# cvg/limap

Hardware: AMD Instinct MI355X
Metric: 3D line candidates scored/sec (100 views x 500 segs per GPU, matched topk=10) (higher is better)
Workload: dtype f64

## Files before the change

limap_amd/csrc/lt_api.cpp:

```cpp

#include "lt_host.h"

using namespace lt;
using namespace lt_impl;

namespace lt_trace {
typedef int (*push_fn)(const char *);
typedef int (*pop_fn)(void);
static push_fn g_push = nullptr;
static pop_fn g_pop = nullptr;
static void init_once() {
  static bool done = false;
  if (done) return;
  done = true;
  const char *sw = getenv("LT_ROCTX");
  if (sw && sw[0] == '0') return;
  const char *libs[] = {"librocprofiler-sdk-roctx.so.1", "librocprofiler-sdk-roctx.so", "libroctx64.so.4", "libroctx64.so"};
  for (const char *l : libs) {
    void *h = dlopen(l, RTLD_LAZY | RTLD_GLOBAL);
    if (!h) continue;
    g_push = (push_fn)dlsym(h, "roctxRangePushA");
    g_pop = (pop_fn)dlsym(h, "roctxRangePop");
    if (g_push && g_pop) return;
    g_push = nullptr;
// ... 508 lines not shown
                    &ctx->d_seg_off, &ctx->d_node_img, &ctx->d_nb_off, &ctx->d_blk_img, &ctx->d_blk_nb,
                    &ctx->d_blk_slot, &ctx->d_blk_order, &ctx->d_m_off, &ctx->d_m_pairs, &ctx->d_c_stream, &ctx->d_ovf, &ctx->d_rowdesc, &ctx->d_pairs,
                    &ctx->d_keys, &ctx->d_rows, &ctx->d_row_blk, &ctx->d_skeys, &ctx->d_srows, &ctx->d_sort_tmp,
                    &ctx->d_conn_off, &ctx->d_st_c, &ctx->d_st_l, &ctx->d_flags, &ctx->d_pos, &ctx->d_scan_tmp,
                    &ctx->d_item_off, &ctx->d_masks, &ctx->d_mask_cnt, &ctx->d_mask_pos, &ctx->d_cand, &ctx->d_hcand, &ctx->d_hlite,
                    &ctx->d_rm_line, &ctx->d_rm_act, &ctx->d_rm_edges, &ctx->d_rm_cnt,
                    &ctx->d_lite, &ctx->d_tri_off, &ctx->d_score, &ctx->d_best_idx, &ctx->d_edge_flag,
                    &ctx->d_nvalid, &ctx->d_edge_off, &ctx->d_edges, &ctx->d_best_c, &ctx->d_best_score,
                    &ctx->d_best_src, &ctx->d_ntris, &ctx->d_err, &ctx->d_blk_line_base, &ctx->d_cnt_bl,
                    &ctx->d_st_key, &ctx->d_wave_count, &ctx->d_wave_pos, &ctx->d_ntris_u, &ctx->d_cand_node,
                    &ctx->d_pair_counter, &ctx->d_result3, &ctx->d_tile_order, &ctx->d_scan_status, &ctx->d_perm, &ctx->d_rng, &ctx->d_chunks, &ctx->d_cand_meta, &ctx->d_st_row, &ctx->d_surv_count, &ctx->d_seg_gates, &ctx->d_blkrec, &ctx->d_seg_vp, &ctx->d_seg_has_vp, &ctx->d_base_bl, &ctx->d_blk_chunk_off, &ctx->d_needed, &ctx->d_seg_pts, &ctx->d_seg_pt_off, &ctx->d_sfm_xyz,
                    &ctx->d_place_perm, &ctx->d_ex_rec, &ctx->d_ex_ent, &ctx->d_node_rec, &ctx->d_ex_z, &ctx->d_tile_list, &ctx->d_tail_keys, &ctx->d_tail_skeys, &ctx->d_tail_sims, &ctx->d_tail_mark,
                    &ctx->d_tail_pos, &ctx->d_tail_recs, &ctx->d_tail_nodes, &ctx->d_tail_tmp, &ctx->d_tail_keep,
                    &ctx->d_tail_kpos, &ctx->d_sp_slots, &ctx->d_sp_cnt, &ctx->d_sp_ovf, &ctx->d_sp_pairs, &ctx->d_sp_desc,
                    &ctx->d_run_len, &ctx->d_slot_row0, &ctx->d_blk_nruns, &ctx->d_ln_flag, &ctx->d_blk_surv, &ctx->d_blk_rnd0,
                    &ctx->d_round_count};
  lt_host::host_block_release(ctx->h_pinned_blk);
  if (ctx->tail_pend.active) lt_host::host_block_release(ctx->tail_pend.hb);
  if (ctx->ev_tail) (void)hipEventDestroy(ctx->ev_tail);
  lt_host::host_block_release(ctx->best_c_blk);
  lt_host::host_block_release(ctx->init_blk);
  for (DevBuf *b : bufs) b->release();
  for (auto &e : ctx->ev_b)
    if (e) (void)hipEventDestroy(e);
  for (auto &e : ctx->ev_end)
    if (e) (void)hipEventDestroy(e);
  if (ctx->pool_stream) (void)hipStreamSynchronize(ctx->pool_stream);
  if (!(ctx->pool_stream && lt_host::stream_set_release(ctx->device, ctx->pool_stream, ctx->ev))) {
    for (auto &ev : ctx->ev)
      if (ev) (void)hipEventDestroy(ev);
    if (ctx->pool_stream) (void)hipStreamDestroy(ctx->pool_stream);
// ... 302 lines not shown
```

limap_amd/csrc/lt_api_run.cpp:

```cpp
#include "lt_host.h"

using namespace lt;
using namespace lt_impl;

extern "C" {

int lt_upload(lt_ctx *ctx) {
  LT_RANGE("lt_upload (match rows + job tables -> HBM)");
  LT_FINISH(ctx);
  if (!ctx->inited) return fail(ctx, LT_ERR_STATE, "upload before Init");
  if (ctx->uploaded) return LT_OK;
  HIPCHK(ctx, hipSetDevice(ctx->device));
  double t0 = now_ms();
  build_job_tables(ctx);
  ctx->blk_vorder_ok = false;
  int rc;
  {
    std::vector<char> need((size_t)std::max(ctx->n_img, 1), 0);
    for (size_t j = 0; j < ctx->job_imgs.size(); ++j) {
      need[(size_t)ctx->job_imgs[j]] = 1;
      for (int nb : ctx->job_nbs[j]) need[(size_t)nb] = 1;
    }
    std::vector<int> list;
    ctx->max_needed_segs = 0;
// ... 85 lines not shown
    }
    if (!ctx->rows_ln)
      launch_expand_rows(ctx->stream, ctx->n_blk, ctx->d_rowdesc.p, ctx->d_c_stream.as<unsigned>(), ctx->d_ovf.as<unsigned>(),
                         ctx->d_m_pairs.as<unsigned>());
    if ((rc = upload_vec(ctx, ctx->d_m_off, m_off))) return rc;
    {
      std::vector<int> vo((size_t)std::max(ctx->n_blk, 1), 0);
      for (int b = 0; b < ctx->n_blk; ++b) vo[(size_t)b] = b;
      std::stable_sort(vo.begin(), vo.begin() + ctx->n_blk, [&](int x, int y) {
        return ctx->h_blk_nb[(size_t)x] != ctx->h_blk_nb[(size_t)y] ? ctx->h_blk_nb[(size_t)x] < ctx->h_blk_nb[(size_t)y]
                                                                    : ctx->h_blk_img[(size_t)x] < ctx->h_blk_img[(size_t)y];
      });
      if ((rc = upload_vec(ctx, ctx->d_blk_vorder, vo))) return rc;
      ctx->blk_vorder_ok = true;
    }
    ENSURE(ctx, ctx->d_blkrec, blk_rec_bytes() * (size_t)std::max(ctx->n_blk, 1));
    launch_build_blk(ctx->stream, ctx->n_blk, ctx->d_m_off.as<long long>(), ctx->d_blk_img.as<int>(),
                     ctx->d_blk_nb.as<int>(), ctx->d_blk_slot.as<int>(), ctx->d_seg_off.as<long long>(),
                     ctx->d_blk_line_base.as<long long>(), ctx->d_blkrec.p);
  } else if (ctx->job_mode == 2) {
    ctx->h_item_off.assign(ctx->G + 1, 0);
    std::vector<int> blk_chunk_off((size_t)std::max(ctx->n_blk, 1), 0);
    ctx->max_chunks = 1;
    long long items = 0, conns = 0;
    for (int i = 0; i < ctx->n_img; ++i) {
      long long per_node = 0, conn_node = 0;
      for (long long b = ctx->h_nb_off[i]; b < ctx->h_nb_off[i + 1]; ++b) {
        int i2 = ctx->h_blk_nb[b];
        long long M2 = ctx->seg_off[i2 + 1] - ctx->seg_off[i2];
        blk_chunk_off[(size_t)b] = (int)per_node;
        ctx->max_chunks = std::max(ctx->max_chunks, (int)((M2 + 63) / 64));
        per_node += (M2 + 63) / 64;
        conn_node += M2;
      }
// ... 205 lines not shown
    const bool fast = ctx->rows_sorted;
    {
      const bool vp_now = ctx->cfg.use_vp && !ctx->cfg.disable_vp_triangulation;
      const bool pts_now = ctx->pts_ready && (!ctx->cfg.disable_many_points_triangulation || !ctx->cfg.disable_one_point_triangulation);
      if (ctx->rows_ln && (vp_now || pts_now)) {
        launch_expand_rows(st, ctx->n_blk, ctx->d_rowdesc.p, ctx->d_c_stream.as<unsigned>(), ctx->d_ovf.as<unsigned>(),
                           ctx->d_m_pairs.as<unsigned>());
        ctx->rows_ln = false;
      }
    }
    const bool ln = ctx->rows_ln && fast;
    const int ln_slots = ln ? ctx->ln_slots : 0;
    if (ln) ENSURE(ctx, ctx->d_round_count, 4 * (size_t)std::max<long long>(ctx->n_round_slots, 1));
    const long long n_waves = (long long)ctx->n_blk * gen_groups(ctx->max_rows);
    const long long n_slots_all = (long long)ctx->n_blk * (ln ? ln_slots : gen_slots(ctx->max_rows));
    const long long n_entries = ctx->h_blk_line_base[ctx->n_blk];
    const bool vp_on = ctx->cfg.use_vp && !ctx->cfg.disable_vp_triangulation;
    if (vp_on && !ctx->vp_ready) return fail(ctx, LT_ERR_STATE, "use_vp is set but InitVPResults was not called");
    const bool pts_any = ctx->pts_ready && (!ctx->cfg.disable_many_points_triangulation || !ctx->cfg.disable_one_point_triangulation);
    const bool many_on = pts_any && !ctx->cfg.disable_many_points_triangulation;
    const bool one_on = pts_any && !ctx->cfg.disable_one_point_triangulation;
    const bool pts_on = pts_any;
    const bool extras = vp_on || pts_on;
    long long staged_total = -1;
    if (!extras) {
      ENSURE(ctx, ctx->d_st_c, sizeof(CRec) * Pn); ENSURE(ctx, ctx->d_st_l, sizeof(double) * Pn);
      ENSURE(ctx, ctx->d_st_key, 4 * (Pn + 64));
    }
    ENSURE(ctx, ctx->d_wave_count, 4 * (size_t)(n_waves + 1));
    if (extras) ENSURE(ctx, ctx->d_wave_pos, 8 * (size_t)(n_waves + 1));
    const long long *group_base = extras ? ctx->d_wave_pos.as<long long>() : nullptr;
// ... 56 lines not shown
          return fail(ctx, LT_ERR_ARGUMENT, "too many candidates in one batch (>= 2^32-1): triangulate the images in smaller batches");
        const size_t Sn = (size_t)std::max<long long>(staged_total, 1);
        ENSURE(ctx, ctx->d_st_c, sizeof(CRec) * Sn); ENSURE(ctx, ctx->d_st_l, sizeof(double) * Sn);
        ENSURE(ctx, ctx->d_st_key, 4 * Sn);
        gen(2);
      }
    }
    bool gen_event_pending = false;
    if (fine_gen && ctx->n_blk > 0 && ctx->max_rows > 0) ev_gen_end = 10;
    else gen_event_pending = true;
    long long *hC = hp;
    long long hC_fallback = 0;
    if (!hC) hC = &hC_fallback;
    if (fast) {
      ENSURE(ctx, ctx->d_node_rec, 16 * (size_t)std::max<long long>(G, 1));
      launch_node_prefix(st, G, ctx->d_node_img.as<int>(), ctx->d_seg_off.as<long long>(),
                         ctx->d_nb_off.as<long long>(), ctx->d_blk_line_base.as<long long>(),
                         ctx->d_cnt_bl.as<unsigned>(), ctx->d_base_bl.as<unsigned>(), ctx->d_ntris_u.as<unsigned>(),
                         ctx->d_tri_off.as<long long>(), ctx->d_scan_status.as<unsigned long long>(),
                         ctx->d_err.as<int>(), ctx->d_node_rec.p);
      node_rec_valid = true;
      ctx->cnt_bl_clean = true;
      const long long bound = P;
      constexpr long long kCountFreeBytes = 48ll << 30;
      const bool perm_bound = !test_switch("LT_TEST_PLACE_COPY");
      const long long per_cand = (perm_bound ? 4 : (long long)(sizeof(CRec) + 8)) + 8 + 4 + 4 + (long long)cand_meta_bytes() +
                                 (long long)score_split_entry_bytes() * 256 / 64;
      if (extras) {
        C_known = staged_total;
      } else if (ctx->h_pinned && bound * per_cand <= kCountFreeBytes && !test_switch("LT_TEST_SYNC_COUNT")) {
        C_known = -1;
        C_bound = bound;
      } else {
// ... 27 lines not shown
        HIPCHK(ctx, hipMemcpyAsync(hC, ctx->d_tri_off.as<long long>() + G, 8, hipMemcpyDeviceToHost, st));
        HIPCHK(ctx, hipStreamSynchronize(st));
        C_known = *hC;
      }
    }
    if (C_known >= 0) C_bound = C_known;
    const size_t Cn = (size_t)std::max<long long>(C_bound, 1);
    if (perm_mode) {
      ENSURE(ctx, ctx->d_place_perm, 4 * Cn);
    } else {
      ENSURE(ctx, ctx->d_cand, sizeof(CRec) * Cn); ENSURE(ctx, ctx->d_lite, sizeof(double) * Cn);
    }
    ENSURE(ctx, ctx->d_score, 8 * Cn); ENSURE(ctx, ctx->d_edge_flag, 4 * Cn); ENSURE(ctx, ctx->d_cand_node, 4 * Cn);
    ctx->cand_cap = (long long)Cn;
    if (fast) {
      launch_place(st, ctx->n_blk, ctx->max_rows, ctx->d_m_off.as<long long>(), ctx->d_blk_img.as<int>(),
                   ctx->d_seg_off.as<long long>(), ctx->d_blk_line_base.as<long long>(),
                   ctx->d_base_bl.as<unsigned>(), ctx->d_wave_count.as<unsigned>(), ctx->d_tri_off.as<long long>(),
                   ctx->d_st_c.as<CRec>(), ctx->d_st_l.as<double>(), ctx->d_st_key.as<unsigned>(),
                   ctx->d_cand.as<CRec>(), ctx->d_lite.as<double>(), ctx->d_cand_node.as<unsigned>(), group_base,
                   perm_mode ? ctx->d_place_perm.as<unsigned>() : nullptr, ctx->d_blk_surv.as<unsigned>(),
                   ctx->d_blk_rnd0.as<unsigned>(), ln ? ctx->d_round_count.as<unsigned>() : nullptr);
    } else {
      ENSURE(ctx, ctx->d_keys, 4 * Cn); ENSURE(ctx, ctx->d_rows, 4 * Cn);
      ENSURE(ctx, ctx->d_skeys, 4 * Cn); ENSURE(ctx, ctx->d_srows, 4 * Cn);
      launch_pack_keys(st, ctx->n_blk, ctx->max_rows, ctx->d_m_off.as<long long>(),
                       ctx->d_wave_count.as<unsigned>(), ctx->d_wave_pos.as<long long>(),
                       ctx->d_st_key.as<unsigned>(), ctx->d_keys.as<unsigned>(), ctx->d_rows.as<unsigned>(), group_base);
      if (C_known > 0) {
        int end_bit = bits_for(G + 1);
        size_t tmp = sort_temp_bytes(C_known, end_bit);
        ENSURE(ctx, ctx->d_sort_tmp, std::max<size_t>(tmp, 16));
// ... 441 lines not shown
```

limap_amd/csrc/lt_ctx.h:

```cpp
#pragma once

#include "../../include/limap_amd.h"
#include "lt_device.h"

#include <algorithm>
#include <cstdlib>
#include <cstring>
#include <mutex>
#include <string>
#include <hip/hip_runtime.h>
#include <unordered_map>
#include <vector>

namespace lt_host {
using namespace lt;

void *dev_block_acquire(size_t bytes, size_t *cap);
void dev_block_release(void *p, size_t cap);

struct DevBuf {
  void *p = nullptr;
  size_t cap = 0;
  DevBuf() = default;
  DevBuf(const DevBuf &) = delete;
// ... 207 lines not shown
  long long max_needed_segs = 0;
  DevBuf d_blk_chunk_off;
  int max_chunks = 1;
  DevBuf d_perm, d_rng;
  DevBuf d_result3;
  DevBuf d_scan_status;
  DevBuf d_tile_order;
  DevBuf d_tile_list;
  DevBuf d_blk_vorder;
  bool blk_vorder_ok = false;
  DevBuf d_pc_cnt, d_pc_list;
  DevBuf d_sp_slots, d_sp_cnt, d_sp_ovf, d_sp_pairs, d_sp_desc;
  bool score_two_kernels = false;
  bool score_fused = false;
  DevBuf d_base_bl;
  DevBuf d_place_perm;
  bool perm_mode = false;
  DevBuf d_ex_rec;
  DevBuf d_node_rec;
  DevBuf d_ex_ent;
  DevBuf d_ex_z;
  long long ex_region_cap = 0;
  double ex_frac = 0.0;
  bool ex_two_pass = false;
  bool ex_staged_set[2] = {false, false};
  bool in_run_async = false;
  bool pend_fine_gen = false, pend_fine_score = false;
  int ex_retry_depth = 0;
  bool host_view_valid = false;
  bool compact_valid = false;
// ... 140 lines not shown
```

limap_amd/csrc/lt_host.h:

```cpp
#pragma once

#include "lt_ctx.h"
#include "lt_tail.h"
#include "lt_rows.h"
#include "lt_pool.h"

#include <algorithm>
#include <atomic>
#include <parallel/algorithm>
#include <chrono>
#include <cmath>
#include <cstdio>
#include <cstring>
#include <dlfcn.h>
#include <map>
#include <mutex>
#include <queue>
#include <set>
#include <string>
#include <unordered_map>
#include <vector>

namespace lt {
void launch_fn_query(hipStream_t st, const double *in30, int by_endpoints, double *out32);
int gen_slots(long long max_rows);
int gen_groups(long long max_rows);
int gen_slots_ln(int max_own_segs);
int gen_max_run();
void launch_rows_ln(hipStream_t st, int n_blk, int n_slots, const void *desc, const unsigned *stream,
                    const long long *blk_line_base, unsigned *rstart, int *blk_nruns, unsigned *run_len,
                    unsigned *slot_row0, unsigned short *tr, int *ln_flag);
size_t seg_gate_bytes();
void launch_build_blk(hipStream_t st, int n_blk, const long long *m_off, const int *blk_img, const int *blk_nb,
                      const int *blk_slot, const long long *seg_off, const long long *blk_line_base, void *blkrec);
size_t blk_rec_bytes();
void launch_gen_split(hipStream_t st, int n_blk, long long max_rows, const GenCfg &cfg, const long long *m_off,
                      const int *m_pairs, const int *blk_img, const int *blk_nb, const int *blk_slot,
                      const long long *seg_off, const Cam *cams, const Seg *segs, const PairRec *pairs,
                      const long long *blk_line_base, CRec *st_r, double *st_unc, unsigned *st_key,
                      unsigned *wave_count, unsigned *cnt_bl, int lds_segs, int lds_segs1, void *st_row,
                      unsigned *surv_count, long long n_segs, void *gates, void *blkrec, hipEvent_t *ev3,
                      const double *seg_vp, const unsigned char *seg_has_vp, const long long *seg_pt_off,
                      const void *seg_pts, const double *sfm_xyz, int *err_flag, int many_on, int one_on,
                      const long long *group_base, int phase, int ln_slots, const unsigned short *tr,
                      const unsigned *run_len, const unsigned *slot_row0, unsigned *blk_surv, const unsigned *blk_rnd0,
                      unsigned *round_count, const int *blk_vorder, unsigned *tri_unit_ctr);
size_t seg_point_bytes();
void launch_node_prefix(hipStream_t st, long long G, const int *node_img, const long long *seg_off,
                        const long long *nb_off, const long long *blk_line_base, unsigned *cnt_bl,
                        unsigned *base_bl, unsigned *n_tris, long long *tri_off, unsigned long long *status,
                        int *err_flag, void *node_rec);
void launch_expand_rows(hipStream_t st, int n_blk, const void *desc, const unsigned *stream, const unsigned *ovf, unsigned *rows);
void launch_place(hipStream_t st, int n_blk, long long max_rows, const long long *m_off, const int *blk_img,
                  const long long *seg_off, const long long *blk_line_base, const unsigned *base_bl,
                  const unsigned *wave_count, const long long *tri_off, const CRec *st_r, const double *st_unc,
                  const unsigned *st_key, CRec *cand, double *cand_unc, unsigned *cand_node, const long long *group_base,
                  unsigned *perm, const unsigned *blk_surv, const unsigned *blk_rnd0, const unsigned *round_count);
void launch_pack_keys(hipStream_t st, int n_blk, long long max_rows, const long long *m_off,
                      const unsigned *wave_count, const long long *wave_pos, const unsigned *st_key,
                      unsigned *keys_c, unsigned *src_c, const long long *group_base);
void launch_permute(hipStream_t st, long long C, const unsigned *skeys, const unsigned *ssrc, const CRec *st_r,
                    const double *st_unc, CRec *cand, double *cand_unc, unsigned *cand_node);
void launch_host_view(hipStream_t st, long long C, const unsigned *perm, const CRec *rec, const double *unc, Cand *out_c,
                      CandLite *out_l);
void launch_cand_node(hipStream_t st, long long G, const long long *tri_off, unsigned *cand_node);
size_t score3_lds_bytes(int max_nb, bool f32);
size_t cand_meta_bytes();
void launch_score3(hipStream_t st, long long C, long long G, const long long *tri_off, const unsigned *cand_node,
                   void *meta, const CRec *cand, const int *node_img, const long long *nb_off,
// ... 57 lines not shown
```

limap_amd/csrc/lt_kernels_v2.hip:

```cpp

#include "lt_devfn.h"

#include <algorithm>

namespace lt {

#ifndef LT_GEN_CHUNKS
#define LT_GEN_CHUNKS 5
#endif
#ifndef LT_GATE_WAVES
#define LT_GATE_WAVES 8
#endif
#ifndef LT_GATE_WAVES_PER_EU
#define LT_GATE_WAVES_PER_EU 4
#endif
#define LT_GATE_OCC __attribute__((amdgpu_waves_per_eu(LT_GATE_WAVES_PER_EU, LT_GATE_WAVES_PER_EU)))
constexpr int kGenChunks = LT_GEN_CHUNKS;
constexpr int kRowsPerWave = 64 * kGenChunks;
constexpr int kGateWaves = LT_GATE_WAVES;
#ifndef LT_TRI_SLOTS
#define LT_TRI_SLOTS 4
#endif
constexpr int kTriSlots = LT_TRI_SLOTS;
#ifndef LT_TRI_WAVES
// ... 47 lines not shown
  const unsigned *slot_row0;
};
static __device__ __forceinline__ long long slot_first_row(const unsigned *__restrict__ slot_row0, int n_slots, int b, int s,
                                                           long long rb) {
  return slot_row0 ? (long long)slot_row0[(size_t)b * n_slots + s] : rb + (long long)s * kRowsPerWave;
}


struct BlkRec {
  long long rb, re;
  long long g1, g2;
  long long lbase;
  int M2;
  int i1, i2, nbslot;
  int M1;
  int pad_;
};
static_assert(sizeof(BlkRec) == 64, "BlkRec layout");

__global__ void k_build_blk(int n_blk, const long long *__restrict__ m_off, const int *__restrict__ blk_img,
                            const int *__restrict__ blk_nb, const int *__restrict__ blk_slot,
                            const long long *__restrict__ seg_off, const long long *__restrict__ blk_line_base,
                            BlkRec *__restrict__ out) {
  int b = blockIdx.x * blockDim.x + threadIdx.x;
  if (b >= n_blk) return;
  BlkRec r;
  r.rb = m_off[b]; r.re = m_off[b + 1];
  r.i1 = blk_img[b]; r.i2 = blk_nb[b]; r.nbslot = blk_slot[b];
  r.g1 = seg_off[r.i1]; r.g2 = seg_off[r.i2];
  r.M2 = (int)(seg_off[r.i2 + 1] - r.g2);
  r.lbase = blk_line_base[b];
  r.M1 = (int)(seg_off[r.i1 + 1] - r.g1);
  r.pad_ = 0;
  out[b] = r;
}

constexpr int kExpandWaves = 4;
__global__ void __launch_bounds__(64 * kExpandWaves)
k_expand_rows(int n_blk, const RowDesc *__restrict__ desc, const unsigned *__restrict__ stream,
              const unsigned *__restrict__ ovf, unsigned *__restrict__ rows) {
  const int b = blockIdx.x;
  if (b >= n_blk) return;
  const RowDesc d = desc[b];
  const int lane = lane_id();
  const int wave = threadIdx.x >> 6;
  unsigned *out = rows + d.row_off;
  if (d.ooff >= 0) {
    for (int r = threadIdx.x; r < d.n; r += 64 * kExpandWaves) out[r] = ovf[d.ooff + r];
// ... 481 lines not shown
  const int n_groups = a.n_slots / kTS;
  const int g = blockIdx.x * kTriWaves + wave;
  if (g >= n_groups) return;
  const BlkRec *rec = blk_r + b;
  const long long rb = rec->rb, re = rec->re;
  const long long r0 = slot_first_row(slot_row0, a.n_slots, b, g * kTS, rb);
  const unsigned lin = (unsigned)b * (unsigned)n_groups + (unsigned)g;
  LT_TRACE_MARK(1, lin, 0);
  if (r0 >= re) {
    if (lane == 0) a.wave_count[lin] = 0;
    return;
  }
  const int i1 = rec->i1, i2 = rec->i2, nbslot = rec->nbslot;
  const long long g1 = rec->g1, g2 = rec->g2;
  const PairRec *pr = pairs_r + b;
  const long long lbase = a.cnt_bl ? rec->lbase : 0;
  const long long out0 = (kExtra && a.group_base) ? a.group_base[lin] : r0;
  const bool wr = !(kExtra && a.count_only);
  unsigned cs[kTS + 1];
  cs[0] = 0;
#pragma unroll
  for (int k = 0; k < kTS; ++k)
    cs[k + 1] = cs[k] + a.surv_count[(size_t)b * a.n_slots + (size_t)g * kTS + k];
  const unsigned n_s = cs[kTS];
  unsigned wcount = 0;
#ifdef LT_TRACE
  if (n_s > 0) LT_TRACE_MARK(1, lin, 1);
#endif
  for (unsigned e0 = 0; e0 < n_s; e0 += 64) {
    const unsigned e = e0 + lane;
    bool ok = false;
// ... 187 lines not shown
    if (!first) v += v_step;
    if (v >= v_end) break;
  }
  first = false;
  const int b = vorder ? vorder[v] : v;
  const int x = x_dyn >= 0 ? x_dyn : (wave + b) % kTriWaves;
  const unsigned n_s = blk_surv[b];
  const int n_rounds = (int)((n_s + 63u) >> 6);
  if (x >= n_rounds) continue;
  const BlkRec *rec = blk_r + b;
  const long long rb = rec->rb;
  const unsigned rnd0 = blk_rnd0[b];
  const int i1 = rec->i1, i2 = rec->i2, nbslot = rec->nbslot;
  const long long g1 = rec->g1, g2 = rec->g2;
  const PairRec *pr = pairs_r + b;
  const long long lbase = rec->lbase;
  for (int r = x; r < n_rounds; r += kTriWaves) {
    LT_TRACE_MARK(1, rnd0 + (unsigned)r, 0);
    const unsigned e = 64u * (unsigned)r + (unsigned)lane;
    bool ok = false;
    GenOut o;
    int line = 0;
    if (e < n_s) {
      const uint2 u = a.st_row[rb + e];
      line = (int)(u.x & 0x7FFFFFFFu);
      const int ng = (int)u.y;
#ifdef LT_TRACE
      if (line >= 0) LT_TRACE_MARK(1, rnd0 + (unsigned)r, 1);
#endif
      const Seg &s1 = a.segs[g1 + line];
      const Seg &s2 = a.segs[g2 + ng];
// ... 22 lines not shown
    wave_lds_sync();
    const long long p0 = rb + 64ll * r;
    double2 *dc = reinterpret_cast<double2 *>(a.st_r + p0);
    for (unsigned u = lane; u < total * 8u; u += 64) dc[u] = Lc[u];
    if ((unsigned)lane < total) {
      a.st_unc[p0 + lane] = Lu[lane];
      a.st_key[p0 + lane] = Lk[lane];
    }
    if (lane == 0) round_count[rnd0 + (unsigned)r] = total;
    wave_lds_sync();
    LT_TRACE_MARK(1, rnd0 + (unsigned)r, 2);
  }
  }
}

#ifndef LT_PLACE_WG_PER_CU
#define LT_PLACE_WG_PER_CU 8
#endif
__global__ void __launch_bounds__(256)
k_place_rounds(const long long *__restrict__ m_off, const int *__restrict__ blk_img, const long long *__restrict__ seg_off,
               const long long *__restrict__ blk_line_base, const unsigned *__restrict__ base_bl,
               const long long *__restrict__ tri_off, const CRec *__restrict__ st_r, const double *__restrict__ st_unc,
               const unsigned *__restrict__ st_key, CRec *__restrict__ cand, double *__restrict__ cand_unc,
               unsigned *__restrict__ cand_node, unsigned *__restrict__ perm, const unsigned *__restrict__ blk_surv,
               const unsigned *__restrict__ blk_rnd0, const unsigned *__restrict__ round_count, int n_blk) {
  const int wave = threadIdx.x >> 6;
  const int lane = lane_id();
  for (int b = (int)blockIdx.x; b < n_blk; b += (int)gridDim.x) {
  const int x = (wave + b) & 3;
  const int n_rounds = (int)((blk_surv[b] + 63u) >> 6);
  if (x >= n_rounds) continue;
  const long long rb = m_off[b];
  const unsigned rnd0 = blk_rnd0[b];
  const long long g1 = seg_off[blk_img[b]];
  const long long lbase = blk_line_base[b];
  unsigned count_n = round_count[rnd0 + (unsigned)x];
  unsigned key_n = st_key[rb + 64ll * x + lane];
  for (int r = x; r < n_rounds; r += 4) {
    const unsigned count = count_n;
    const unsigned key_raw = key_n;
    if (r + 4 < n_rounds) {
      count_n = round_count[rnd0 + (unsigned)(r + 4)];
      key_n = st_key[rb + 64ll * (r + 4) + lane];
    }
    if (count == 0) continue;
    const long long s0 = rb + 64ll * r;
    const bool act = (unsigned)lane < count;
    const unsigned key = act ? key_raw : 0xFFFFFFFFu;
    const unsigned prev = (unsigned)__shfl_up((int)key, 1);
    const bool head = act && (lane == 0 || key != prev);
    const unsigned long long heads = __ballot(head);
    const int my_head = 63 - __builtin_clzll(heads & ((2ull << lane) - 1ull) | 1ull);
    const unsigned key0 = (unsigned)__builtin_amdgcn_readfirstlane((int)key);
    unsigned carry = 0;
    for (int pr_ = r - 1; pr_ >= 0; --pr_) {
      const unsigned pc = round_count[rnd0 + (unsigned)pr_];
      if (pc == 0) continue;
      const long long j = (long long)pc - 64 + lane;
      const bool valid = j >= 0;
      const unsigned k = valid ? st_key[rb + 64ll * pr_ + j] : 0u;
      const unsigned long long m = __ballot(valid && k == key0);
      const unsigned lead = m == ~0ull ? 64u : (unsigned)__builtin_clzll(~m);
      carry += lead;
      if (lead < pc) break;
    }
    unsigned pos32 = 0;
    if (act) {
      const unsigned rank = (unsigned)(lane - my_head) + (my_head == 0 ? carry : 0u);
      const long long pos = tri_off[key] + base_bl[lbase + (long long)(key - g1)] + rank;
      pos32 = (unsigned)pos;
      cand_node[pos] = key;
      if (perm) perm[pos] = (unsigned)(s0 + lane);
    }
    if (perm) continue;
    const double2 *src_c = reinterpret_cast<const double2 *>(st_r + s0);
    double2 *dst_c = reinterpret_cast<double2 *>(cand);
#pragma unroll
    for (int it = 0; it < 8; ++it) {
      const unsigned u = (unsigned)it * 64u + (unsigned)lane;
      const unsigned ci = u >> 3, piece = u & 7u;
      const unsigned p = (unsigned)__shfl((int)pos32, (int)ci);
      if (u < count * 8u) dst_c[(size_t)p * 8u + piece] = src_c[u];
    }
    if (act) cand_unc[pos32] = st_unc[s0 + lane];
  }
  }
}

__global__ void __launch_bounds__(256)
k_node_prefix(long long G, const int *__restrict__ node_img, const long long *__restrict__ seg_off,
              const long long *__restrict__ nb_off, const long long *__restrict__ blk_line_base,
              unsigned *__restrict__ cnt_bl, unsigned *__restrict__ base_bl, unsigned *__restrict__ n_tris,
              long long *__restrict__ tri_off, unsigned long long *__restrict__ status, int *__restrict__ err_flag,
              uint4 *__restrict__ node_rec) {
  __shared__ unsigned s_tile;
  __shared__ long long s_wave[4];
  __shared__ long long s_prefix;
  if (threadIdx.x == 0) s_tile = (unsigned)atomicAdd(&status[0], 1ull);
  __syncthreads();
  const long long tile = s_tile;
  const long long g = tile * 256 + threadIdx.x;
  const int lane = lane_id(), wave = threadIdx.x >> 6;
  unsigned run = 0;
  unsigned nbv = 0;
  if (g < G) {
    int img = node_img[g];
    int line = (int)(g - seg_off[img]);
    const long long b0 = nb_off[img], b1 = nb_off[img + 1];
    nbv = ((unsigned)b0 << 8) | (unsigned)(b1 - b0);
    for (long long bb = b0; bb < b1; bb += 16) {
      long long e[16];
      unsigned c[16];
#pragma unroll
      for (int k = 0; k < 16; ++k) {
        e[k] = (bb + k < b1) ? blk_line_base[bb + k] + line : -1;
      }
#pragma unroll
      for (int k = 0; k < 16; ++k) c[k] = e[k] >= 0 ? cnt_bl[e[k]] : 0u;
#pragma unroll
      for (int k = 0; k < 16; ++k) {
        if (e[k] >= 0) {
          cnt_bl[e[k]] = 0;
          base_bl[e[k]] = run;
        }
        run += c[k];
      }
    }
  }
  long long incl = (long long)run;
#pragma unroll
  for (int d = 1; d < 64; d <<= 1) {
    const long long o = __shfl_up(incl, d);
    if (lane >= d) incl += o;
  }
  if (lane == 63) s_wave[wave] = incl;
  __syncthreads();
  long long wbase = 0;
  for (int w = 0; w < wave; ++w) wbase += s_wave[w];
// ... 31 lines not shown
      atomicExch(&status[1 + tile], (2ull << 62) | (unsigned long long)(prefix + total));
      s_prefix = prefix;
    }
  }
  __syncthreads();
  const long long off = s_prefix + wbase + incl - (long long)run;
  if (g <= G) {
    tri_off[g] = off;
    n_tris[g] = run;
  }
  if (node_rec && g < G) node_rec[g] = uint4{(unsigned)(off & 0xFFFFFFFFll), (unsigned)(off >> 32), run, nbv};
}

template <int kTS>
__global__ void __launch_bounds__(256)
k_place(const long long *__restrict__ m_off, const int *__restrict__ blk_img,
        const long long *__restrict__ seg_off, const long long *__restrict__ blk_line_base,
        const unsigned *__restrict__ base_bl, const unsigned *__restrict__ wave_count,
        const long long *__restrict__ tri_off, const CRec *__restrict__ st_r,
        const double *__restrict__ st_unc, const unsigned *__restrict__ st_key, CRec *__restrict__ cand,
        double *__restrict__ cand_unc, unsigned *__restrict__ cand_node, int n_groups,
        const long long *__restrict__ group_base, unsigned *__restrict__ perm,
        const unsigned *__restrict__ slot_row0) {
  const int wave = threadIdx.x >> 6;
  const int lane = lane_id();
  const int b = blockIdx.y;
  const int g = blockIdx.x * 4 + wave;
  if (g >= n_groups) return;
  const int n_slots = n_groups * kTS;
  const long long rb = m_off[b], re = m_off[b + 1];
  const long long r0 = slot_first_row(slot_row0, n_slots, b, g * kTS, rb);
  if (r0 >= re) return;
  const unsigned lin = (unsigned)b * (unsigned)n_groups + (unsigned)g;
  const unsigned count = wave_count[lin];
  if (count == 0) return;
  const long long g1 = seg_off[blk_img[b]];
  const long long lbase = blk_line_base[b];
  const long long s0 = group_base ? group_base[lin] : r0;
  static_assert(sizeof(CRec) == 8 * 16, "record size in 16-byte units");
  for (unsigned e0 = 0; e0 < count; e0 += 64) {
    const unsigned e = e0 + lane;
    const bool act = e < count;
    unsigned pos32 = 0;
    const unsigned key = act ? st_key[s0 + e] : 0xFFFFFFFFu;
    const unsigned prev = (unsigned)__shfl_up((int)key, 1);
    const bool head = act && (lane == 0 || key != prev);
    const unsigned long long heads = __ballot(head);
    const int my_head = 63 - __builtin_clzll(heads & ((2ull << lane) - 1ull) | 1ull);
    const unsigned key0 = (unsigned)__builtin_amdgcn_readfirstlane((int)key);
    unsigned carry = 0;
    {
      long long cur_r0 = r0;
// ... 12 lines not shown
          const long long n_valid = idx_end < 64 ? idx_end : 64;
          if ((long long)lead < n_valid) { more = false; break; }
          idx_end -= n_valid;
        }
        if (!more) break;
        if (cur_g == 0) break;
        cur_g -= 1;
        cur_r0 = slot_first_row(slot_row0, n_slots, b, cur_g * kTS, rb);
        cur_lin -= 1;
        idx_end = (long long)wave_count[cur_lin];
      }
    }
    if (act) {
      const unsigned rank = (unsigned)(lane - my_head) + (my_head == 0 ? carry : 0u);
      const long long toff = tri_off[key];
      const long long pos = toff + base_bl[lbase + (long long)(key - g1)] + rank;
      pos32 = (unsigned)pos;
      cand_node[pos] = key;
      if (perm) perm[pos] = (unsigned)(s0 + e);
    }
    if (perm) continue;
    const unsigned nb = min(64u, count - e0);
    const double2 *src_c = reinterpret_cast<const double2 *>(st_r + s0 + e0);
    double2 *dst_c = reinterpret_cast<double2 *>(cand);
#pragma unroll
    for (int it = 0; it < 8; ++it) {
      const unsigned u = (unsigned)it * 64u + (unsigned)lane;
      const unsigned ci = u >> 3, piece = u & 7u;
      const unsigned p = (unsigned)__shfl((int)pos32, (int)ci);
      if (u < nb * 8u) dst_c[(size_t)p * 8u + piece] = src_c[u];
    }
// ... 74 lines not shown
int score_read_trace(unsigned long long *host, size_t n);
extern "C" int lt_debug_read_trace(unsigned long long *host, size_t n) {
  const int rc = (int)hipMemcpyFromSymbol(host, HIP_SYMBOL(g_trace), n * 8, 0, hipMemcpyDeviceToHost);
  return rc ? rc : score_read_trace(host, n);
}
#endif
size_t seg_gate_bytes() { return sizeof(SegGate); }
size_t seg_point_bytes() { return sizeof(SegPoint); }
size_t blk_rec_bytes() { return sizeof(BlkRec); }
void launch_expand_rows(hipStream_t st, int n_blk, const void *desc, const unsigned *stream, const unsigned *ovf, unsigned *rows) {
  if (n_blk > 0)
    hipLaunchKernelGGL(k_expand_rows, dim3((unsigned)n_blk), dim3(64 * kExpandWaves), 0, st, n_blk, reinterpret_cast<const RowDesc *>(desc), stream,
                       ovf, rows);
}
void launch_build_blk(hipStream_t st, int n_blk, const long long *m_off, const int *blk_img, const int *blk_nb,
                      const int *blk_slot, const long long *seg_off, const long long *blk_line_base, void *blkrec) {
  if (n_blk > 0)
    hipLaunchKernelGGL(k_build_blk, dim3(nblk2(n_blk, 128)), dim3(128), 0, st, n_blk, m_off, blk_img, blk_nb, blk_slot,
                       seg_off, blk_line_base, reinterpret_cast<BlkRec *>(blkrec));
}
void launch_gen_split(hipStream_t st, int n_blk, long long max_rows, const GenCfg &cfg, const long long *m_off,
                      const int *m_pairs, const int *blk_img, const int *blk_nb, const int *blk_slot,
                      const long long *seg_off, const Cam *cams, const Seg *segs, const PairRec *pairs,
                      const long long *blk_line_base, CRec *st_r, double *st_unc, unsigned *st_key,
                      unsigned *wave_count, unsigned *cnt_bl, int lds_segs, int lds_segs1, void *st_row,
                      unsigned *surv_count, long long n_segs, void *gates, void *blkrec, hipEvent_t *ev3,
                      const double *seg_vp, const unsigned char *seg_has_vp, const long long *seg_pt_off,
                      const void *seg_pts, const double *sfm_xyz, int *err_flag, int many_on, int one_on,
                      const long long *group_base, int phase, int ln_slots, const unsigned short *tr,
                      const unsigned *run_len, const unsigned *slot_row0, unsigned *blk_surv, const unsigned *blk_rnd0,
                      unsigned *round_count, const int *blk_vorder, unsigned *tri_unit_ctr) {
  if (n_blk <= 0 || max_rows <= 0) return;
  static int n_cu = 0;
  if (n_cu == 0) {
// ... 44 lines not shown
  const size_t tri_lds = kTriWaves * (64 * 9 + 16) * sizeof(double2);
  if (ln) {
    const dim3 tg((unsigned)std::min<long long>(n_blk, (long long)n_cu * (16 / kTriWaves)));
    hipLaunchKernelGGL(k_tri_rounds, tg, dim3(64 * kTriWaves), tri_lds, st, a, cfg, a.cams, a.pairs, a.blk, blk_surv, blk_rnd0,
                       round_count, blk_vorder, tri_unit_ctr);
  } else {
    const dim3 tg(nblk2(a.n_slots / kTriSlots, kTriWaves), n_blk);
    if (extra)
      hipLaunchKernelGGL((k_tri_rows<true, kTriSlots>), tg, dim3(64 * kTriWaves), 0, st, a, cfg, a.cams, a.pairs, a.blk, a.slot_row0);
    else
      hipLaunchKernelGGL((k_tri_rows<false, kTriSlots>), tg, dim3(64 * kTriWaves), tri_lds, st, a, cfg, a.cams, a.pairs, a.blk,
                         a.slot_row0);
  }
  if (ev3 && phase != 1) (void)hipEventRecord(ev3[2], st);
}
void launch_node_prefix(hipStream_t st, long long G, const int *node_img, const long long *seg_off,
                        const long long *nb_off, const long long *blk_line_base, unsigned *cnt_bl,
                        unsigned *base_bl, unsigned *n_tris, long long *tri_off, unsigned long long *status,
                        int *err_flag, void *node_rec) {
  hipLaunchKernelGGL(k_node_prefix, dim3(nblk2(G + 1, 256)), dim3(256), 0, st, G, node_img, seg_off, nb_off,
                     blk_line_base, cnt_bl, base_bl, n_tris, tri_off, status, err_flag, reinterpret_cast<uint4 *>(node_rec));
}
void launch_place(hipStream_t st, int n_blk, long long max_rows, const long long *m_off, const int *blk_img,
                  const long long *seg_off, const long long *blk_line_base, const unsigned *base_bl,
                  const unsigned *wave_count, const long long *tri_off, const CRec *st_r, const double *st_unc,
                  const unsigned *st_key, CRec *cand, double *cand_unc, unsigned *cand_node, const long long *group_base,
                  unsigned *perm, const unsigned *blk_surv, const unsigned *blk_rnd0, const unsigned *round_count) {
  if (n_blk <= 0 || max_rows <= 0) return;
  if (round_count) {
    static int n_cu = 0;
    if (n_cu == 0) {
      int dev = 0;
      if (hipGetDevice(&dev) != hipSuccess ||
          hipDeviceGetAttribute(&n_cu, hipDeviceAttributeMultiprocessorCount, dev) != hipSuccess || n_cu <= 0)
        n_cu = 256;
    }
    hipLaunchKernelGGL(k_place_rounds, dim3((unsigned)std::min<long long>(n_blk, (long long)n_cu * LT_PLACE_WG_PER_CU)), dim3(256), 0, st, m_off,
                       blk_img, seg_off, blk_line_base, base_bl, tri_off, st_r, st_unc, st_key, cand, cand_unc, cand_node, perm,
                       blk_surv, blk_rnd0, round_count, n_blk);
    return;
  }
  const int n_groups = gen_groups(max_rows);
  hipLaunchKernelGGL(k_place<kTriSlots>, dim3(nblk2(n_groups, 4), n_blk), dim3(256), 0, st, m_off, blk_img, seg_off,
                     blk_line_base, base_bl, wave_count, tri_off, st_r, st_unc, st_key, cand, cand_unc, cand_node, n_groups,
                     group_base, perm, (const unsigned *)nullptr);
}
void launch_pack_keys(hipStream_t st, int n_blk, long long max_rows, const long long *m_off,
                      const unsigned *wave_count, const long long *wave_pos, const unsigned *st_key,
                      unsigned *keys_c, unsigned *src_c, const long long *group_base) {
  if (n_blk <= 0 || max_rows <= 0) return;
  const int n_groups = gen_groups(max_rows);
  hipLaunchKernelGGL(k_pack_keys, dim3(nblk2(n_groups, 4), n_blk), dim3(256), 0, st, m_off, wave_count, wave_pos,
                     st_key, keys_c, src_c, n_groups, group_base);
}
void launch_permute(hipStream_t st, long long C, const unsigned *skeys, const unsigned *ssrc, const CRec *st_r,
                    const double *st_unc, CRec *cand, double *cand_unc, unsigned *cand_node) {
  if (C > 0)
    hipLaunchKernelGGL(k_permute, dim3(nblk2(C, 256)), dim3(256), 0, st, C, skeys, ssrc, st_r, st_unc, cand, cand_unc,
                       cand_node);
// ... 7 lines not shown
```

Baseline: 2.500 billion.

## Re-lay per-(neighbour,segment) counters as slot-major strided arrays and restructure placement

Changes the counter/base arrays from per-block line-base layout to a neighbour-slot-major layout with a padded global-segment stride, so node_prefix reads coalesced contiguous columns per slot. A per-node neighbour descriptor is precomputed on the host and uploaded, which drops the indirect node_img/seg_off/nb_off lookups. k_place_rounds moves from a persistent grid-stride loop with 4 waves to one workgroup per block with 16 waves. Each round now prefetches the previous round's keys for the carry computation. The trade-off is a counter buffer sized max_nb*stride, which may be larger than before, plus a new 2^32 limit check.

```diff
diff --git a/limap_amd/csrc/lt_api.cpp b/limap_amd/csrc/lt_api.cpp
--- a/limap_amd/csrc/lt_api.cpp
+++ b/limap_amd/csrc/lt_api.cpp
@@ -546,7 +546,7 @@
                     &ctx->d_tail_pos, &ctx->d_tail_recs, &ctx->d_tail_nodes, &ctx->d_tail_tmp, &ctx->d_tail_keep,
                     &ctx->d_tail_kpos, &ctx->d_sp_slots, &ctx->d_sp_cnt, &ctx->d_sp_ovf, &ctx->d_sp_pairs, &ctx->d_sp_desc,
                     &ctx->d_run_len, &ctx->d_slot_row0, &ctx->d_blk_nruns, &ctx->d_ln_flag, &ctx->d_blk_surv, &ctx->d_blk_rnd0,
-                    &ctx->d_round_count};
+                    &ctx->d_round_count, &ctx->d_node_nbv};
   lt_host::host_block_release(ctx->h_pinned_blk);
   if (ctx->tail_pend.active) lt_host::host_block_release(ctx->tail_pend.hb);
   if (ctx->ev_tail) (void)hipEventDestroy(ctx->ev_tail);
diff --git a/limap_amd/csrc/lt_api_run.cpp b/limap_amd/csrc/lt_api_run.cpp
--- a/limap_amd/csrc/lt_api_run.cpp
+++ b/limap_amd/csrc/lt_api_run.cpp
@@ -123,10 +123,21 @@
       if ((rc = upload_vec(ctx, ctx->d_blk_vorder, vo))) return rc;
       ctx->blk_vorder_ok = true;
     }
+    {
+      ctx->cnt_stride = (std::max<long long>(ctx->G, 1) + 255) & ~255ll;
+      if ((long long)ctx->max_nb * ctx->cnt_stride >= (1ll << 32))
+        return fail(ctx, LT_ERR_ARGUMENT, "too many (neighbour, segment) counters in one batch (>= 2^32): triangulate the images in smaller batches");
+      std::vector<unsigned> nbv((size_t)std::max<long long>(ctx->G, 1), 0u);
+      for (long long g = 0; g < ctx->G; ++g) {
+        const int i = ctx->h_node_img[(size_t)g];
+        nbv[(size_t)g] = ((unsigned)ctx->h_nb_off[i] << 8) | (unsigned)(ctx->h_nb_off[i + 1] - ctx->h_nb_off[i]);
+      }
+      if ((rc = upload_vec(ctx, ctx->d_node_nbv, nbv))) return rc;
+    }
     ENSURE(ctx, ctx->d_blkrec, blk_rec_bytes() * (size_t)std::max(ctx->n_blk, 1));
     launch_build_blk(ctx->stream, ctx->n_blk, ctx->d_m_off.as<long long>(), ctx->d_blk_img.as<int>(),
                      ctx->d_blk_nb.as<int>(), ctx->d_blk_slot.as<int>(), ctx->d_seg_off.as<long long>(),
-                     ctx->d_blk_line_base.as<long long>(), ctx->d_blkrec.p);
+                     ctx->d_blk_line_base.as<long long>(), ctx->cnt_stride, ctx->d_blkrec.p);
   } else if (ctx->job_mode == 2) {
     ctx->h_item_off.assign(ctx->G + 1, 0);
     std::vector<int> blk_chunk_off((size_t)std::max(ctx->n_blk, 1), 0);
@@ -362,7 +373,7 @@
     if (ln) ENSURE(ctx, ctx->d_round_count, 4 * (size_t)std::max<long long>(ctx->n_round_slots, 1));
     const long long n_waves = (long long)ctx->n_blk * gen_groups(ctx->max_rows);
     const long long n_slots_all = (long long)ctx->n_blk * (ln ? ln_slots : gen_slots(ctx->max_rows));
-    const long long n_entries = ctx->h_blk_line_base[ctx->n_blk];
+    const long long n_entries = (long long)ctx->max_nb * ctx->cnt_stride;
     const bool vp_on = ctx->cfg.use_vp && !ctx->cfg.disable_vp_triangulation;
     if (vp_on && !ctx->vp_ready) return fail(ctx, LT_ERR_STATE, "use_vp is set but InitVPResults was not called");
     const bool pts_any = ctx->pts_ready && (!ctx->cfg.disable_many_points_triangulation || !ctx->cfg.disable_one_point_triangulation);
@@ -449,9 +460,7 @@
     if (!hC) hC = &hC_fallback;
     if (fast) {
       ENSURE(ctx, ctx->d_node_rec, 16 * (size_t)std::max<long long>(G, 1));
-      launch_node_prefix(st, G, ctx->d_node_img.as<int>(), ctx->d_seg_off.as<long long>(),
-                         ctx->d_nb_off.as<long long>(), ctx->d_blk_line_base.as<long long>(),
-                         ctx->d_cnt_bl.as<unsigned>(), ctx->d_base_bl.as<unsigned>(), ctx->d_ntris_u.as<unsigned>(),
+      launch_node_prefix(st, G, ctx->cnt_stride, ctx->d_node_nbv.as<unsigned>(), ctx->d_cnt_bl.as<unsigned>(), ctx->d_base_bl.as<unsigned>(), ctx->d_ntris_u.as<unsigned>(),
                          ctx->d_tri_off.as<long long>(), ctx->d_scan_status.as<unsigned long long>(),
                          ctx->d_err.as<int>(), ctx->d_node_rec.p);
       node_rec_valid = true;
@@ -509,8 +518,7 @@
     ENSURE(ctx, ctx->d_score, 8 * Cn); ENSURE(ctx, ctx->d_edge_flag, 4 * Cn); ENSURE(ctx, ctx->d_cand_node, 4 * Cn);
     ctx->cand_cap = (long long)Cn;
     if (fast) {
-      launch_place(st, ctx->n_blk, ctx->max_rows, ctx->d_m_off.as<long long>(), ctx->d_blk_img.as<int>(),
-                   ctx->d_seg_off.as<long long>(), ctx->d_blk_line_base.as<long long>(),
+      launch_place(st, ctx->n_blk, ctx->max_rows, ctx->d_m_off.as<long long>(), ctx->d_blk_slot.as<int>(), ctx->cnt_stride,
                    ctx->d_base_bl.as<unsigned>(), ctx->d_wave_count.as<unsigned>(), ctx->d_tri_off.as<long long>(),
                    ctx->d_st_c.as<CRec>(), ctx->d_st_l.as<double>(), ctx->d_st_key.as<unsigned>(),
                    ctx->d_cand.as<CRec>(), ctx->d_lite.as<double>(), ctx->d_cand_node.as<unsigned>(), group_base,
diff --git a/limap_amd/csrc/lt_ctx.h b/limap_amd/csrc/lt_ctx.h
--- a/limap_amd/csrc/lt_ctx.h
+++ b/limap_amd/csrc/lt_ctx.h
@@ -245,6 +245,8 @@
   bool score_two_kernels = false;
   bool score_fused = false;
   DevBuf d_base_bl;
+  long long cnt_stride = 0;
+  DevBuf d_node_nbv;
   DevBuf d_place_perm;
   bool perm_mode = false;
   DevBuf d_ex_rec;
diff --git a/limap_amd/csrc/lt_host.h b/limap_amd/csrc/lt_host.h
--- a/limap_amd/csrc/lt_host.h
+++ b/limap_amd/csrc/lt_host.h
@@ -32,7 +32,8 @@
                     unsigned *slot_row0, unsigned short *tr, int *ln_flag);
 size_t seg_gate_bytes();
 void launch_build_blk(hipStream_t st, int n_blk, const long long *m_off, const int *blk_img, const int *blk_nb,
-                      const int *blk_slot, const long long *seg_off, const long long *blk_line_base, void *blkrec);
+                      const int *blk_slot, const long long *seg_off, const long long *blk_line_base, long long cnt_stride,
+                      void *blkrec);
 size_t blk_rec_bytes();
 void launch_gen_split(hipStream_t st, int n_blk, long long max_rows, const GenCfg &cfg, const long long *m_off,
                       const int *m_pairs, const int *blk_img, const int *blk_nb, const int *blk_slot,
@@ -46,13 +47,12 @@
                       const unsigned *run_len, const unsigned *slot_row0, unsigned *blk_surv, const unsigned *blk_rnd0,
                       unsigned *round_count, const int *blk_vorder, unsigned *tri_unit_ctr);
 size_t seg_point_bytes();
-void launch_node_prefix(hipStream_t st, long long G, const int *node_img, const long long *seg_off,
-                        const long long *nb_off, const long long *blk_line_base, unsigned *cnt_bl,
+void launch_node_prefix(hipStream_t st, long long G, long long cnt_stride, const unsigned *node_nbv, unsigned *cnt_bl,
                         unsigned *base_bl, unsigned *n_tris, long long *tri_off, unsigned long long *status,
                         int *err_flag, void *node_rec);
 void launch_expand_rows(hipStream_t st, int n_blk, const void *desc, const unsigned *stream, const unsigned *ovf, unsigned *rows);
-void launch_place(hipStream_t st, int n_blk, long long max_rows, const long long *m_off, const int *blk_img,
-                  const long long *seg_off, const long long *blk_line_base, const unsigned *base_bl,
+void launch_place(hipStream_t st, int n_blk, long long max_rows, const long long *m_off, const int *blk_slot,
+                  long long cnt_stride, const unsigned *base_bl,
                   const unsigned *wave_count, const long long *tri_off, const CRec *st_r, const double *st_unc,
                   const unsigned *st_key, CRec *cand, double *cand_unc, unsigned *cand_node, const long long *group_base,
                   unsigned *perm, const unsigned *blk_surv, const unsigned *blk_rnd0, const unsigned *round_count);
diff --git a/limap_amd/csrc/lt_kernels_v2.hip b/limap_amd/csrc/lt_kernels_v2.hip
--- a/limap_amd/csrc/lt_kernels_v2.hip
+++ b/limap_amd/csrc/lt_kernels_v2.hip
@@ -85,14 +85,14 @@
   int M2;
   int i1, i2, nbslot;
   int M1;
-  int pad_;
+  unsigned cbase;
 };
 static_assert(sizeof(BlkRec) == 64, "BlkRec layout");
 
 __global__ void k_build_blk(int n_blk, const long long *__restrict__ m_off, const int *__restrict__ blk_img,
                             const int *__restrict__ blk_nb, const int *__restrict__ blk_slot,
                             const long long *__restrict__ seg_off, const long long *__restrict__ blk_line_base,
-                            BlkRec *__restrict__ out) {
+                            long long cnt_stride, BlkRec *__restrict__ out) {
   int b = blockIdx.x * blockDim.x + threadIdx.x;
   if (b >= n_blk) return;
   BlkRec r;
@@ -102,7 +102,7 @@
   r.M2 = (int)(seg_off[r.i2 + 1] - r.g2);
   r.lbase = blk_line_base[b];
   r.M1 = (int)(seg_off[r.i1 + 1] - r.g1);
-  r.pad_ = 0;
+  r.cbase = (unsigned)((long long)r.nbslot * cnt_stride + r.g1);
   out[b] = r;
 }
 
@@ -614,7 +614,7 @@
   const int i1 = rec->i1, i2 = rec->i2, nbslot = rec->nbslot;
   const long long g1 = rec->g1, g2 = rec->g2;
   const PairRec *pr = pairs_r + b;
-  const long long lbase = a.cnt_bl ? rec->lbase : 0;
+  const long long lbase = a.cnt_bl ? (long long)rec->cbase : 0;
   const long long out0 = (kExtra && a.group_base) ? a.group_base[lin] : r0;
   const bool wr = !(kExtra && a.count_only);
   unsigned cs[kTS + 1];
@@ -832,7 +832,7 @@
   const int i1 = rec->i1, i2 = rec->i2, nbslot = rec->nbslot;
   const long long g1 = rec->g1, g2 = rec->g2;
   const PairRec *pr = pairs_r + b;
-  const long long lbase = rec->lbase;
+  const long long lbase = (long long)rec->cbase;
   for (int r = x; r < n_rounds; r += kTriWaves) {
     LT_TRACE_MARK(1, rnd0 + (unsigned)r, 0);
     const unsigned e = 64u * (unsigned)r + (unsigned)lane;
@@ -885,37 +885,36 @@
   }
 }
 
-#ifndef LT_PLACE_WG_PER_CU
-#define LT_PLACE_WG_PER_CU 8
-#endif
-__global__ void __launch_bounds__(256)
-k_place_rounds(const long long *__restrict__ m_off, const int *__restrict__ blk_img, const long long *__restrict__ seg_off,
-               const long long *__restrict__ blk_line_base, const unsigned *__restrict__ base_bl,
-               const long long *__restrict__ tri_off, const CRec *__restrict__ st_r, const double *__restrict__ st_unc,
+#ifndef LT_PLACE_WAVES
+#define LT_PLACE_WAVES 16
+#endif
+constexpr int kPlaceWaves = LT_PLACE_WAVES;
+__global__ void __launch_bounds__(64 * kPlaceWaves)
+k_place_rounds(const long long *__restrict__ m_off, const int *__restrict__ blk_slot, long long cnt_stride,
+               const unsigned *__restrict__ base_bl, const long long *__restrict__ tri_off,
+               const CRec *__restrict__ st_r, const double *__restrict__ st_unc,
                const unsigned *__restrict__ st_key, CRec *__restrict__ cand, double *__restrict__ cand_unc,
                unsigned *__restrict__ cand_node, unsigned *__restrict__ perm, const unsigned *__restrict__ blk_surv,
                const unsigned *__restrict__ blk_rnd0, const unsigned *__restrict__ round_count, int n_blk) {
-  const int wave = threadIdx.x >> 6;
+  const int wave = __builtin_amdgcn_readfirstlane((int)(threadIdx.x >> 6));
   const int lane = lane_id();
-  for (int b = (int)blockIdx.x; b < n_blk; b += (int)gridDim.x) {
-  const int x = (wave + b) & 3;
+  const int b = (int)blockIdx.x;
+  if (b >= n_blk) return;
   const int n_rounds = (int)((blk_surv[b] + 63u) >> 6);
-  if (x >= n_rounds) continue;
+  if (wave >= n_rounds) return;
   const long long rb = m_off[b];
   const unsigned rnd0 = blk_rnd0[b];
-  const long long g1 = seg_off[blk_img[b]];
-  const long long lbase = blk_line_base[b];
-  unsigned count_n = round_count[rnd0 + (unsigned)x];
-  unsigned key_n = st_key[rb + 64ll * x + lane];
-  for (int r = x; r < n_rounds; r += 4) {
-    const unsigned count = count_n;
-    const unsigned key_raw = key_n;
-    if (r + 4 < n_rounds) {
-      count_n = round_count[rnd0 + (unsigned)(r + 4)];
-      key_n = st_key[rb + 64ll * (r + 4) + lane];
+  const unsigned *__restrict__ bl = base_bl + (long long)blk_slot[b] * cnt_stride;
+  for (int r = wave; r < n_rounds; r += kPlaceWaves) {
+    const long long s0 = rb + 64ll * r;
+    const unsigned count = round_count[rnd0 + (unsigned)r];
+    const unsigned key_raw = st_key[s0 + lane];
+    unsigned pc = 0, pk = 0;
+    if (r > 0) {
+      pc = round_count[rnd0 + (unsigned)(r - 1)];
+      pk = st_key[s0 - 64 + lane];
     }
     if (count == 0) continue;
-    const long long s0 = rb + 64ll * r;
     const bool act = (unsigned)lane < count;
     const unsigned key = act ? key_raw : 0xFFFFFFFFu;
     const unsigned prev = (unsigned)__shfl_up((int)key, 1);
@@ -924,21 +923,27 @@
     const int my_head = 63 - __builtin_clzll(heads & ((2ull << lane) - 1ull) | 1ull);
     const unsigned key0 = (unsigned)__builtin_amdgcn_readfirstlane((int)key);
     unsigned carry = 0;
-    for (int pr_ = r - 1; pr_ >= 0; --pr_) {
-      const unsigned pc = round_count[rnd0 + (unsigned)pr_];
-      if (pc == 0) continue;
-      const long long j = (long long)pc - 64 + lane;
+    bool further = r > 0;
+    if (pc > 0) {
+      const unsigned long long m = __ballot((unsigned)lane < pc && pk == key0) << (64u - pc);
+      carry = m == ~0ull ? 64u : (unsigned)__builtin_clzll(~m);
+      further = carry == pc;
+    }
+    for (int pr_ = r - 2; further && pr_ >= 0; --pr_) {
+      const unsigned qc = round_count[rnd0 + (unsigned)pr_];
+      if (qc == 0) continue;
+      const long long j = (long long)qc - 64 + lane;
       const bool valid = j >= 0;
       const unsigned k = valid ? st_key[rb + 64ll * pr_ + j] : 0u;
       const unsigned long long m = __ballot(valid && k == key0);
       const unsigned lead = m == ~0ull ? 64u : (unsigned)__builtin_clzll(~m);
       carry += lead;
-      if (lead < pc) break;
+      further = lead == qc;
     }
     unsigned pos32 = 0;
     if (act) {
       const unsigned rank = (unsigned)(lane - my_head) + (my_head == 0 ? carry : 0u);
-      const long long pos = tri_off[key] + base_bl[lbase + (long long)(key - g1)] + rank;
+      const long long pos = tri_off[key] + bl[key] + rank;
       pos32 = (unsigned)pos;
       cand_node[pos] = key;
       if (perm) perm[pos] = (unsigned)(s0 + lane);
@@ -955,12 +960,10 @@
     }
     if (act) cand_unc[pos32] = st_unc[s0 + lane];
   }
-  }
 }
 
 __global__ void __launch_bounds__(256)
-k_node_prefix(long long G, const int *__restrict__ node_img, const long long *__restrict__ seg_off,
-              const long long *__restrict__ nb_off, const long long *__restrict__ blk_line_base,
+k_node_prefix(long long G, long long cnt_stride, const unsigned *__restrict__ node_nbv,
               unsigned *__restrict__ cnt_bl, unsigned *__restrict__ base_bl, unsigned *__restrict__ n_tris,
               long long *__restrict__ tri_off, unsigned long long *__restrict__ status, int *__restrict__ err_flag,
               uint4 *__restrict__ node_rec) {
@@ -969,30 +972,25 @@
   __shared__ long long s_prefix;
   if (threadIdx.x == 0) s_tile = (unsigned)atomicAdd(&status[0], 1ull);
   __syncthreads();
-  const long long tile = s_tile;
+  const long long tile = (long long)(unsigned)__builtin_amdgcn_readfirstlane((int)s_tile);
   const long long g = tile * 256 + threadIdx.x;
   const int lane = lane_id(), wave = threadIdx.x >> 6;
   unsigned run = 0;
   unsigned nbv = 0;
   if (g < G) {
-    int img = node_img[g];
-    int line = (int)(g - seg_off[img]);
-    const long long b0 = nb_off[img], b1 = nb_off[img + 1];
-    nbv = ((unsigned)b0 << 8) | (unsigned)(b1 - b0);
-    for (long long bb = b0; bb < b1; bb += 16) {
-      long long e[16];
-      unsigned c[16];
-#pragma unroll
-      for (int k = 0; k < 16; ++k) {
-        e[k] = (bb + k < b1) ? blk_line_base[bb + k] + line : -1;
-      }
-#pragma unroll
-      for (int k = 0; k < 16; ++k) c[k] = e[k] >= 0 ? cnt_bl[e[k]] : 0u;
-#pragma unroll
-      for (int k = 0; k < 16; ++k) {
-        if (e[k] >= 0) {
-          cnt_bl[e[k]] = 0;
-          base_bl[e[k]] = run;
+    nbv = node_nbv[g];
+    unsigned *__restrict__ ct = cnt_bl + tile * 256;
+    unsigned *__restrict__ bt = base_bl + tile * 256;
+    const int n = (int)(nbv & 0xFFu);
+    for (int k0 = 0; k0 < n; k0 += 32) {
+      unsigned c[32];
+#pragma unroll
+      for (int k = 0; k < 32; ++k) c[k] = (k0 + k < n) ? (ct + (long long)(k0 + k) * cnt_stride)[threadIdx.x] : 0u;
+#pragma unroll
+      for (int k = 0; k < 32; ++k) {
+        if (k0 + k < n) {
+          (ct + (long long)(k0 + k) * cnt_stride)[threadIdx.x] = 0;
+          (bt + (long long)(k0 + k) * cnt_stride)[threadIdx.x] = run;
         }
         run += c[k];
       }
@@ -1054,8 +1052,7 @@
 
 template <int kTS>
 __global__ void __launch_bounds__(256)
-k_place(const long long *__restrict__ m_off, const int *__restrict__ blk_img,
-        const long long *__restrict__ seg_off, const long long *__restrict__ blk_line_base,
+k_place(const long long *__restrict__ m_off, const int *__restrict__ blk_slot, long long cnt_stride,
         const unsigned *__restrict__ base_bl, const unsigned *__restrict__ wave_count,
         const long long *__restrict__ tri_off, const CRec *__restrict__ st_r,
         const double *__restrict__ st_unc, const unsigned *__restrict__ st_key, CRec *__restrict__ cand,
@@ -1074,8 +1071,7 @@
   const unsigned lin = (unsigned)b * (unsigned)n_groups + (unsigned)g;
   const unsigned count = wave_count[lin];
   if (count == 0) return;
-  const long long g1 = seg_off[blk_img[b]];
-  const long long lbase = blk_line_base[b];
+  const unsigned *__restrict__ bl = base_bl + (long long)blk_slot[b] * cnt_stride;
   const long long s0 = group_base ? group_base[lin] : r0;
   static_assert(sizeof(CRec) == 8 * 16, "record size in 16-byte units");
   for (unsigned e0 = 0; e0 < count; e0 += 64) {
@@ -1118,7 +1114,7 @@
     if (act) {
       const unsigned rank = (unsigned)(lane - my_head) + (my_head == 0 ? carry : 0u);
       const long long toff = tri_off[key];
-      const long long pos = toff + base_bl[lbase + (long long)(key - g1)] + rank;
+      const long long pos = toff + bl[key] + rank;
       pos32 = (unsigned)pos;
       cand_node[pos] = key;
       if (perm) perm[pos] = (unsigned)(s0 + e);
@@ -1223,10 +1219,11 @@
                        ovf, rows);
 }
 void launch_build_blk(hipStream_t st, int n_blk, const long long *m_off, const int *blk_img, const int *blk_nb,
-                      const int *blk_slot, const long long *seg_off, const long long *blk_line_base, void *blkrec) {
+                      const int *blk_slot, const long long *seg_off, const long long *blk_line_base, long long cnt_stride,
+                      void *blkrec) {
   if (n_blk > 0)
     hipLaunchKernelGGL(k_build_blk, dim3(nblk2(n_blk, 128)), dim3(128), 0, st, n_blk, m_off, blk_img, blk_nb, blk_slot,
-                       seg_off, blk_line_base, reinterpret_cast<BlkRec *>(blkrec));
+                       seg_off, blk_line_base, cnt_stride, reinterpret_cast<BlkRec *>(blkrec));
 }
 void launch_gen_split(hipStream_t st, int n_blk, long long max_rows, const GenCfg &cfg, const long long *m_off,
                       const int *m_pairs, const int *blk_img, const int *blk_nb, const int *blk_slot,
@@ -1301,35 +1298,26 @@
   }
   if (ev3 && phase != 1) (void)hipEventRecord(ev3[2], st);
 }
-void launch_node_prefix(hipStream_t st, long long G, const int *node_img, const long long *seg_off,
-                        const long long *nb_off, const long long *blk_line_base, unsigned *cnt_bl,
+void launch_node_prefix(hipStream_t st, long long G, long long cnt_stride, const unsigned *node_nbv, unsigned *cnt_bl,
                         unsigned *base_bl, unsigned *n_tris, long long *tri_off, unsigned long long *status,
                         int *err_flag, void *node_rec) {
-  hipLaunchKernelGGL(k_node_prefix, dim3(nblk2(G + 1, 256)), dim3(256), 0, st, G, node_img, seg_off, nb_off,
-                     blk_line_base, cnt_bl, base_bl, n_tris, tri_off, status, err_flag, reinterpret_cast<uint4 *>(node_rec));
-}
-void launch_place(hipStream_t st, int n_blk, long long max_rows, const long long *m_off, const int *blk_img,
-                  const long long *seg_off, const long long *blk_line_base, const unsigned *base_bl,
+  hipLaunchKernelGGL(k_node_prefix, dim3(nblk2(G + 1, 256)), dim3(256), 0, st, G, cnt_stride, node_nbv, cnt_bl, base_bl, n_tris, tri_off, status, err_flag, reinterpret_cast<uint4 *>(node_rec));
+}
+void launch_place(hipStream_t st, int n_blk, long long max_rows, const long long *m_off, const int *blk_slot,
+                  long long cnt_stride, const unsigned *base_bl,
                   const unsigned *wave_count, const long long *tri_off, const CRec *st_r, const double *st_unc,
                   const unsigned *st_key, CRec *cand, double *cand_unc, unsigned *cand_node, const long long *group_base,
                   unsigned *perm, const unsigned *blk_surv, const unsigned *blk_rnd0, const unsigned *round_count) {
   if (n_blk <= 0 || max_rows <= 0) return;
   if (round_count) {
-    static int n_cu = 0;
-    if (n_cu == 0) {
-      int dev = 0;
-      if (hipGetDevice(&dev) != hipSuccess ||
-          hipDeviceGetAttribute(&n_cu, hipDeviceAttributeMultiprocessorCount, dev) != hipSuccess || n_cu <= 0)
-        n_cu = 256;
-    }
-    hipLaunchKernelGGL(k_place_rounds, dim3((unsigned)std::min<long long>(n_blk, (long long)n_cu * LT_PLACE_WG_PER_CU)), dim3(256), 0, st, m_off,
-                       blk_img, seg_off, blk_line_base, base_bl, tri_off, st_r, st_unc, st_key, cand, cand_unc, cand_node, perm,
-                       blk_surv, blk_rnd0, round_count, n_blk);
+    hipLaunchKernelGGL(k_place_rounds, dim3((unsigned)n_blk), dim3(64 * kPlaceWaves), 0, st, m_off, blk_slot, cnt_stride,
+                       base_bl, tri_off, st_r, st_unc, st_key, cand, cand_unc, cand_node, perm, blk_surv, blk_rnd0,
+                       round_count, n_blk);
     return;
   }
   const int n_groups = gen_groups(max_rows);
-  hipLaunchKernelGGL(k_place<kTriSlots>, dim3(nblk2(n_groups, 4), n_blk), dim3(256), 0, st, m_off, blk_img, seg_off,
-                     blk_line_base, base_bl, wave_count, tri_off, st_r, st_unc, st_key, cand, cand_unc, cand_node, n_groups,
+  hipLaunchKernelGGL(k_place<kTriSlots>, dim3(nblk2(n_groups, 4), n_blk), dim3(256), 0, st, m_off, blk_slot, cnt_stride,
+                     base_bl, wave_count, tri_off, st_r, st_unc, st_key, cand, cand_unc, cand_node, n_groups,
                      group_base, perm, (const unsigned *)nullptr);
 }
 void launch_pack_keys(hipStream_t st, int n_blk, long long max_rows, const long long *m_off,
```

Result: no change. 2.511 billion (median of 5 runs) (+0.4%).
